# adama-wzr/EffectiveDiffusivityFVM

Hardware: AMD Instinct MI355X
Metric: Mcells*iter/s (Jacobi sweep) at 4096^2 (higher is better)
Workload: dtype f64

## Files before the change

### effectivediffusivityfvm_amd/_capi.py

```python
import ctypes as C
import os

import numpy as np

_PKG = os.path.dirname(os.path.abspath(__file__))
LIB_PATH = os.environ.get("DEFF_AMD_LIB") or os.path.join(_PKG, "libdeff_amd.so")

KERNEL_AUTO, KERNEL_EXPLICIT, KERNEL_SCALAR, KERNEL_MATFREE, KERNEL_MATFREE_TB = range(5)
KERNEL_NAMES = {"auto": 0, "explicit": 1, "scalar": 2, "matfree": 3, "matfree_tb": 4}

SYMBOLS = [
    "deff_version", "deff_last_error", "deff_error_string", "deff_device_count",
    "deff_create", "deff_create_batch", "deff_batch_size", "deff_recommended_batch", "deff_destroy", "deff_mesh", "deff_set_kernel", "deff_get_kernel",
    "deff_set_tuning", "deff_get_plan", "deff_set_image", "deff_synth_image", "deff_get_image",
    "deff_load_jpeg_gray", "deff_free", "deff_assemble_2phase", "deff_assemble_3phase", "deff_flood_fill", "deff_assemble_from_D", "deff_set_system", "deff_get_system",
    "deff_init_linear", "deff_set_field", "deff_get_field", "deff_solve", "deff_solve_batch", "deff_solve_cg", "deff_sweeps",
    "deff_slab_group_create", "deff_slab_group_destroy", "deff_slab_group_layout", "deff_slab_group_set_tuning", "deff_slab_group_get_plan",
    "deff_slab_group_set_image", "deff_slab_group_synth_image", "deff_slab_group_assemble_2phase",
    "deff_slab_group_init_linear", "deff_slab_group_set_field", "deff_slab_group_get_field",
    "deff_slab_group_sweeps", "deff_slab_group_flux", "deff_slab_group_solve",
    "deff_rccl_unique_id", "deff_slab_rank_create", "deff_slab_rank_create_custom", "deff_slab_rank_destroy", "deff_slab_rank_layout",
    "deff_slab_rank_window", "deff_slab_rank_context", "deff_slab_rank_set_tuning", "deff_slab_rank_set_image_window",
    "deff_slab_rank_synth_image", "deff_slab_rank_assemble_3phase", "deff_slab_group_assemble_3phase", "deff_slab_rank_get_field", "deff_slab_rank_sweeps", "deff_slab_rank_solve",
    "deff_solve_stream", "deff_get_slot_field", "deff_debug_tb_stamps", "deff_flux", "deff_residual", "deff_residual_slot", "deff_residual_D", "deff_set_progress", "deff_last_launches", "deff_device_field", "deff_synchronize",
]


class DeffError(RuntimeError):
    def __init__(self, code, msg):
        super().__init__(f"deff_amd error {code}: {msg}")
        self.code = code


class Result(C.Structure):
    _fields_ = [("iters", C.c_int64), ("checks", C.c_int64), ("deff_raw", C.c_double),
                ("conv", C.c_double), ("loop_ms", C.c_double)]


class CGResultC(C.Structure):
    _fields_ = [("iters", C.c_int64), ("rel_residual", C.c_double), ("deff_raw", C.c_double),
                ("loop_ms", C.c_double), ("converged", C.c_int)]


PROGRESS_FN = C.CFUNCTYPE(None, C.c_int64, C.c_double, C.c_double, C.c_void_p)
NEXT_IMAGE_FN = C.CFUNCTYPE(C.c_int, C.c_void_p, C.c_int, C.POINTER(C.c_uint8), C.POINTER(C.c_int64))
IMAGE_DONE_FN = C.CFUNCTYPE(None, C.c_void_p, C.c_int64, C.c_int, C.POINTER(Result))
_cdp = C.POINTER(C.c_double)
# ... 78 lines not shown
    L.deff_slab_group_solve.argtypes = [ctx, C.c_double, C.c_double, C.c_int64, C.c_int64, C.POINTER(Result),
                                        C.c_void_p, C.c_void_p]
    L.deff_rccl_unique_id.argtypes = [C.c_char_p]
    L.deff_slab_rank_create.argtypes = [C.c_int, C.c_int, C.c_int, C.c_int, C.c_int, C.c_char_p, C.POINTER(ctx)]
    L.deff_slab_rank_create_custom.argtypes = [C.c_int, C.c_int, C.c_int, C.c_int, C.c_int, HOST_EXCHANGE_FN,
                                               HOST_ALLGATHER_FN, C.c_void_p, C.POINTER(ctx)]
    L.deff_slab_rank_destroy.argtypes = [ctx]
    L.deff_slab_rank_layout.argtypes = [ctx, ip, ip]
    L.deff_slab_rank_window.argtypes = [ctx, ip, ip]
    L.deff_slab_rank_context.argtypes = [ctx, C.POINTER(ctx)]
    L.deff_slab_rank_set_image_window.argtypes = [ctx, _u8p]
    L.deff_slab_rank_synth_image.argtypes = [ctx, C.c_uint64, C.c_uint64]
    L.deff_slab_rank_assemble_3phase.argtypes = [ctx, C.c_double, C.c_double, C.c_double, C.c_void_p, C.c_double, C.c_double]
    L.deff_slab_group_assemble_3phase.argtypes = [ctx, C.c_double, C.c_double, C.c_double, C.c_void_p, C.c_double, C.c_double]
    L.deff_slab_rank_get_field.argtypes = [ctx, _dp]
    L.deff_slab_rank_sweeps.argtypes = [ctx, C.c_int64, C.c_double, C.POINTER(C.c_float)]
    L.deff_slab_rank_solve.argtypes = [ctx, C.c_double, C.c_double, C.c_int64, C.c_int64, C.POINTER(Result),
                                       C.c_void_p, C.c_void_p]
    L.deff_solve_stream.argtypes = [ctx, C.c_int, C.c_int, C.c_int, C.c_int, C.c_double, C.c_double, C.c_double,
                                    C.c_double, C.c_double, C.c_double, C.c_int64, C.c_int64, NEXT_IMAGE_FN,
                                    IMAGE_DONE_FN, C.c_void_p]
    L.deff_get_slot_field.argtypes = [ctx, C.c_int, _dp]
    L.deff_debug_tb_stamps.argtypes = [ctx, C.c_double, C.c_void_p, C.POINTER(C.c_int)]
    L.deff_device_field.argtypes = [ctx, C.POINTER(C.c_void_p), C.POINTER(C.c_size_t)]
    L.deff_synchronize.argtypes = [ctx]
    _lib = L
    return L


def check(rc):
    if rc != 0:
        raise DeffError(rc, load().deff_last_error().decode("utf-8", "replace"))
```

### effectivediffusivityfvm_amd/csrc/api_core.hip

```cpp
#include "ctx.hpp"
#include <algorithm>
#include "driver/jpeg_gray.hpp"
#include "flood_fill.hpp"


thread_local char g_err[512] = "";

int fail(int code, const char *fmt, ...)
{
    va_list ap;
    va_start(ap, fmt);
    vsnprintf(g_err, sizeof g_err, fmt, ap);
    va_end(ap);
    return code;
}


extern "C" const char *deff_version(void) { return "deff_amd 0.1 (gfx950)"; }
extern "C" const char *deff_last_error(void) { return g_err; }
extern "C" const char *deff_error_string(int code)
{
    switch (code) {
    case DEFF_OK: return "ok";
    case DEFF_EINVAL: return "invalid argument";
// ... 68 lines not shown
        }
    } while (0);
    if (rc != DEFF_OK) return rc;
    resident_chain_ctx_created(device);
    c->chain_counted = true;
    guard.c = nullptr;
    *out = c;
    return DEFF_OK;
}
DEFF_API_CATCH

extern "C" int deff_destroy(deff_ctx *c)
try {
    if (!c) return DEFF_OK;
    (void)hipSetDevice(c->device);
    if (c->stream) (void)hipStreamSynchronize(c->stream);
    void *bufs[] = {c->pix, c->a0, c->c0, c->aW, c->aE, c->aS, c->aN, c->b, c->code, c->lut,
                    c->Dl, c->Dr, c->mf, c->x[0], c->x[1], c->scratch, c->active};
    for (void *p : bufs) if (p) (void)hipFree(p);
    if (c->mf_host) (void)hipHostFree(c->mf_host);
    if (c->q) (void)hipFree(c->q);
    if (c->resid) (void)hipFree(c->resid);
    if (c->tb_dealt) (void)hipFree(c->tb_dealt);
    if (c->res_flags) (void)hipFree(c->res_flags);
    if (c->res_abort) (void)hipFree(c->res_abort);
    if (c->res_backup) (void)hipFree(c->res_backup);
    void *cg_bufs[] = {c->cg_r, c->cg_p[0], c->cg_p[1], c->cg_tab, c->cg_part, c->cg_scal, c->cg_flags};
    for (void *p : cg_bufs) if (p) (void)hipFree(p);
    if (c->cg_ev0) (void)hipEventDestroy(c->cg_ev0);
    if (c->cg_ev1) (void)hipEventDestroy(c->cg_ev1);
    if (c->q_host) (void)hipHostFree(c->q_host);
    if (c->chain_counted) resident_chain_ctx_destroyed(c->device);
    if (c->ev0) (void)hipEventDestroy(c->ev0);
    if (c->ev1) (void)hipEventDestroy(c->ev1);
    if (c->stream) (void)hipStreamDestroy(c->stream);
    delete c;
    return DEFF_OK;
}
DEFF_API_CATCH

extern "C" int deff_mesh(const deff_ctx *c, int *nx, int *ny, double *dx, double *dy)
try {
    if (!c) return fail(DEFF_EINVAL, "ctx is NULL");
    if (nx) *nx = c->nxt;
    if (ny) *ny = c->ny;
    if (dx) *dx = c->dx;
// ... 95 lines not shown
    else if (!strcmp(key, "tb_R")) c->tb_R = value;
    else if (!strcmp(key, "tb_debug_stall")) c->tb_debug_stall = value;
    else if (!strcmp(key, "tb_debug_stall_skip")) c->tb_debug_stall_skip = value;
    else if (!strcmp(key, "res_kt")) c->res_kt = value;
    else if (!strcmp(key, "tb_sym")) c->tb_sym = value;
    else if (!strcmp(key, "tb_launch")) {
        if (value > 1) return fail(DEFF_EINVAL, "tb_launch takes 0 (resident passes where the tiles fit the chip) or 1 (one launch per pass)");
        c->tb_resident = value == 1 ? 0 : 1;
    }
    else if (!strcmp(key, "flux_reduce")) c->flux_reduce = value > 2 ? 0 : value;
    else if (!strcmp(key, "tb_NW")) c->tb_NW = value;
    else if (!strcmp(key, "dict")) c->dict_enabled = value ? 1 : 0;
    else if (!strcmp(key, "tb_xmajor")) c->tb_xmajor = value ? 1 : 0;
    else if (!strcmp(key, "fma")) c->fma = value ? 1 : 0;
    else if (!strcmp(key, "tb_wall_halo")) c->tb_wall_halo = value > 2 ? 2 : value;
    else if (!strcmp(key, "tb_wg")) c->tb_wg = (value + 7) / 8 * 8;
    else if (!strcmp(key, "tb_ranked")) { c->tb_ranked = value ? 1 : 0; c->tb_rank_lost = 0; }
    else if (!strcmp(key, "tb_tall_deal")) c->tb_tall_deal = value ? 1 : 0;
    else if (!strcmp(key, "tb_sym_age")) c->tb_sym_age = value ? 1 : 0;
    else if (!strcmp(key, "tb_sym_shape")) c->tb_sym_shape = value;
    else if (!strcmp(key, "tb_rank_w0")) c->tb_rank_w[0] = value;
    else if (!strcmp(key, "tb_rank_w1")) c->tb_rank_w[1] = value;
    else if (!strcmp(key, "tb_rank_w2")) c->tb_rank_w[2] = value;
    else if (!strcmp(key, "tb_rank_wall")) c->tb_rank_wall = value;
    else return fail(DEFF_EINVAL, "unknown tuning key '%s'", key);
    return DEFF_OK;
}
DEFF_API_CATCH

extern "C" int deff_get_plan(deff_ctx *c, const char *key, int *value)
try {
    if (!c || !key || !value) return fail(DEFF_EINVAL, "NULL argument");
    if (!strcmp(key, "tb_T")) *value = c->plan_T;
    else if (!strcmp(key, "tb_LY")) *value = c->plan_LY;
    else if (!strcmp(key, "tb_strips")) *value = c->plan_ntx;
    else if (!strcmp(key, "tb_chunks_per_image")) *value = c->plan_cpi;
    else if (!strcmp(key, "tb_blocks")) *value = c->plan_blocks;
    else if (!strcmp(key, "tb_impl")) *value = c->plan_impl;
    else if (!strcmp(key, "tb_R")) *value = c->plan_R;
    else if (!strcmp(key, "tb_resident")) *value = c->plan_resident;
    else if (!strcmp(key, "tb_sym")) *value = c->links_sym;
    else if (!strcmp(key, "tb_NW")) *value = c->plan_NW;
    else if (!strcmp(key, "tb_fallbacks")) *value = c->res_fallbacks;
    else if (!strcmp(key, "tb_ranked")) *value = c->plan_ranked;
    else if (!strcmp(key, "tb_aged")) *value = c->plan_aged;
    else if (!strcmp(key, "tb_rank_misses")) *value = c->tb_rank_misses;
    else if (!strcmp(key, "tb_rank_lost")) *value = c->tb_rank_lost;
    else return fail(DEFF_EINVAL, "unknown plan key '%s'", key);
    return DEFF_OK;
}
DEFF_API_CATCH


int image_shape(deff_ctx *c, int W, int H, int ampX, int ampY)
{
    if (W < 1 || H < 1 || ampX < 1 || ampY < 1)
        return fail(DEFF_EINVAL, "image %dx%d / mesh amplification %dx%d invalid", W, H, ampX, ampY);
    if ((long long)W * ampX != c->nxt || (long long)H * ampY != c->ny)
        return fail(DEFF_EINVAL, "image %dx%d x amp %dx%d does not match mesh %dx%d", W, H, ampX, ampY,
                    c->nxt, c->ny);
    if (c->pix && (c->W != W || c->H != H)) { HIP_TRY(hipFree(c->pix)); c->pix = nullptr; }
    TRY(dev_alloc(&c->pix, (size_t)W * H * c->nimg));
    c->W = W; c->H = H; c->ampX = ampX; c->ampY = ampY;
    return DEFF_OK;
}

extern "C" int deff_set_image(deff_ctx *c, const uint8_t *pix, int W, int H, int ampX, int ampY)
try {
    if (!c || !pix) return fail(DEFF_EINVAL, "NULL argument");
    TRY(use_device(c));
// ... 379 lines not shown
```

### effectivediffusivityfvm_amd/csrc/api_solve.hip

```cpp
#include "ctx.hpp"
#include "kernels_dict.hpp"
#include "kernels_sweep.hpp"
#include "kernels_tb.hpp"
#include "kernels_wgtile.hpp"
#include <array>
#include <map>
#include <mutex>



template <class Make> static constexpr auto by_flag(Make make) { return std::array{make(TbTag<false>{}), make(TbTag<true>{})}; }
template <class Make> static constexpr auto by_flags(Make make)
{
    return std::array{make(TbTag<false>{}, TbTag<false>{}), make(TbTag<false>{}, TbTag<true>{}), make(TbTag<true>{}, TbTag<false>{}),
                      make(TbTag<true>{}, TbTag<true>{})};
}
template <class E, size_t... N> static constexpr auto cat(const std::array<E, N> &...parts)
{
    std::array<E, (N + ...)> all{};
    size_t k = 0;
    auto put = [&](const auto &part) { for (const E &e : part) all[k++] = e; };
    (put(parts), ...);
    return all;
}
// ... 494 lines not shown
    if (!found) return DEFF_OK;
    TRY(check_links_symmetric(c));
    if (c->links_sym == 1) *sym = found;
    return DEFF_OK;
}

static int plan_sym(deff_ctx *c, SweepPlan *pl, int T, int own_h, const TileKernel *tile)
{
    pl->impl = 2;
    pl->tile = tile;
    const int lymax = tile->tile_rows() - 2 * T;
    const int cpi = (own_h + lymax - 1) / lymax;
    pl->LY = (own_h + cpi - 1) / cpi;
    pl->tcpi = (own_h + pl->LY - 1) / pl->LY;
    pl->tgy = pl->tcpi * c->nimg;
    const long tiles = (long)pl->ntx * pl->tgy;
    pl->tgx = (int)tiles;
    pl->tblocks = (int)(((tiles + 7) / 8) * 8);
    pl->resident = true;
    TRY(ensure_resident_buffers(c, tiles));
    return DEFF_OK;
}

static int deal_ranked_tiles(deff_ctx *c, SweepPlan *pl, int T, int own_lo, int own_h, int resident, bool *dealt)
{
    *dealt = false;
    int cus = 0;
    HIP_TRY(hipDeviceGetAttribute(&cus, hipDeviceAttributeMultiprocessorCount, c->device));
    const int xcds = 8, per_xcd = cus / xcds, occ = cus > 0 ? resident / cus : 0;
    if (cus % xcds != 0 || occ != 3 || resident != occ * cus) return DEFF_OK;
    const int slots = cus * 4;
    const int ntx = pl->ntx, cap = own_h / (3 * T);
    const int ncol = ntx * c->nimg;
    if (ntx > 0xFFFF || c->nimg > 0x7FFF || ncol > slots) return DEFF_OK;
    const int nq = std::min(slots / ncol, cap);
    if (nq < 1 || c->tb_rank_wall < 1000 || c->tb_rank_w[0] < 1 || c->tb_rank_w[1] < 1 || c->tb_rank_w[2] < 1) return DEFF_OK;
    const std::vector<int> key = {T, own_lo, own_h, ntx, c->nimg, pl->shift, resident, c->tb_rank_w[0], c->tb_rank_w[1], c->tb_rank_w[2], c->tb_rank_wall};
    auto fill_plan = [&]() {
        pl->dealt = c->tb_dealt;
        pl->LY = c->tb_dealt_LY;
        pl->tcpi = 3 * c->tb_dealt_nmax;
        pl->tgy = pl->tcpi * c->nimg;
        pl->tgx = (ntx * pl->tgy + 3) / 4;
        pl->tblocks = resident;
        *dealt = true;
    };
    if (c->tb_dealt && key == c->tb_dealt_key) { fill_plan(); return DEFF_OK; }
    const double v[3] = {(double)c->tb_rank_w[0], (double)c->tb_rank_w[1], (double)c->tb_rank_w[2]};
    const int K = T * (T - 1) + 8;
    std::vector<std::array<double, 3>> speed(ncol, std::array<double, 3>{v[0], v[1], v[2]});
    const bool walls = ntx >= 3;
    if (walls) {
        const int hw = (T + 1) & ~1, wout = TB_COLS - 2 * hw;
        const int last_cols = c->nx - ((ntx - 1) * wout - pl->shift);
        const double extra = c->tb_rank_wall / 1000.0 - 1.0, by_rank[3] = {2.5, 1.5, 1.0};
        const double fill = (double)std::min(last_cols, TB_COLS) / TB_COLS;
        for (int img = 0; img < c->nimg; ++img)
            for (int r = 0; r < 3; ++r) {
                speed[(size_t)img * ntx][r] = v[r] / (1.0 + extra * by_rank[r]);
                speed[(size_t)img * ntx + ntx - 1][r] = v[r] / (1.0 + extra * by_rank[r] * fill);
            }
    }
    struct Strip { int n[3]; int ly[3]; };
    std::vector<Strip> st(ncol);
    for (auto &q : st) q.n[0] = q.n[1] = q.n[2] = nq;
    int spare[3] = {slots - ncol * nq, slots - ncol * nq, slots - ncol * nq};
    auto strip_time = [&](int tx) {
        const Strip &q = st[tx];
        const std::array<double, 3> &u = speed[tx];
        return ((double)T * own_h + (double)K * (q.n[0] + q.n[1] + q.n[2])) / (q.n[0] * u[0] + q.n[1] * u[1] + q.n[2] * u[2]);
    };
    for (int it = 0; it < 3 * slots; ++it) {
        int worst = -1;
        double tw = 0;
        for (int tx = 0; tx < ncol; ++tx) {
            const double t = strip_time(tx);
            if (t > tw) { tw = t; worst = tx; }
        }
        int r = -1;
        for (int k = 0; k < 3; ++k)
            if (spare[k] > 0 && st[worst].n[k] < cap && (r < 0 || spare[k] > spare[r])) r = k;
        if (r < 0) break;
        ++st[worst].n[r];
        --spare[r];
    }
    int nmax = 0;
    for (int tx = 0; tx < ncol; ++tx) {
        Strip &q = st[tx];
        const double t = strip_time(tx);
        int left = own_h;
        for (int r = 2; r >= 1; --r) {
            int ly = (int)((t * speed[tx][r] - K) / T);
            if (ly < T) ly = T;
            q.ly[r] = ly;
            left -= q.n[r] * ly;
        }
        q.ly[0] = (left + q.n[0] - 1) / q.n[0];
        if (q.ly[0] < T) return DEFF_OK;
        nmax = std::max(nmax, std::max(q.n[0], std::max(q.n[1], q.n[2])));
    }
    if ((long)3 * c->nimg * ntx * nmax >= (1L << 30)) return DEFF_OK;
    const size_t entries = (size_t)resident * 4 + 1;
    {
        std::vector<int4> &tab = c->tb_dealt_host;
        tab.assign(entries, make_int4(0, 0, 0, 0));
        auto tile = [&](int r, int col, int q) {
            const Strip &sp = st[col];
            const int img = col / ntx, tx = col % ntx;
            const int own0 = own_lo + img * c->ny;
            const int own_hi = own0 + own_h;
            int ry0 = own0;
            for (int k = 0; k < r; ++k) ry0 += sp.n[k] * sp.ly[k];
            ry0 += q * sp.ly[r];
            int rows_here = std::min(sp.ly[r], own_hi - ry0);
            if (r == 2 && q == sp.n[2] - 1) rows_here = own_hi - ry0;
            return make_int4(tx | (img << 16), ry0, rows_here > 0 ? rows_here : 0, (int)((unsigned)(((r * c->nimg + img) * ntx + tx) * nmax + q) | ((unsigned)r << 30)));
        };
        for (int r = 0; r < 3; ++r) {
            auto slot = [&](int m, int w) { return ((((size_t)(r * per_xcd + m % per_xcd) << 3) | (size_t)(m / per_xcd)) * 4 + w); };
            std::vector<char> used((size_t)cus * 4, 0);
            std::vector<int4> wall_tiles;
            if (walls)
                for (int img = 0; img < c->nimg; ++img)
                    for (int tx : {0, ntx - 1})
                        for (int q = 0; q < st[(size_t)img * ntx + tx].n[r]; ++q) wall_tiles.push_back(tile(r, img * ntx + tx, q));
            const int nw = (int)wall_tiles.size();
            for (int k = 0; k < nw; ++k) {
                int m = (int)(((long)k * cus) / std::max(nw, 1) + (long)r * cus / 3) % cus, w = 0;
                while (used[(size_t)m * 4 + w]) { if (++w == 4) { w = 0; m = (m + 1) % cus; } }
                used[(size_t)m * 4 + w] = 1;
                tab[slot(m, w)] = wall_tiles[k];
            }
            int m = 0, w = 0;
            for (int col = 0; col < ncol; ++col) {
                if (walls && (col % ntx == 0 || col % ntx == ntx - 1)) continue;
                for (int q = 0; q < st[col].n[r]; ++q) {
                    while (m < cus && used[(size_t)m * 4 + w]) { if (++w == 4) { w = 0; ++m; } }
                    if (m >= cus) return fail(DEFF_ESTATE, "dealt tiles: more chunks than waves (rank %d)", r);
                    used[(size_t)m * 4 + w] = 1;
                    tab[slot(m, w)] = tile(r, col, q);
                }
            }
        }
        if (c->tb_dealt_cap < entries) {
            TRY(resident_check(c));
            if (c->tb_dealt) { HIP_TRY(hipStreamSynchronize(c->stream)); HIP_TRY(hipFree(c->tb_dealt)); c->tb_dealt = nullptr; }
            HIP_TRY(hipMalloc((void **)&c->tb_dealt, entries * sizeof(int4)));
            c->tb_dealt_cap = entries;
        }
        HIP_TRY(hipMemcpyAsync(c->tb_dealt, tab.data(), entries * sizeof(int4), hipMemcpyHostToDevice, c->stream));
        HIP_TRY(hipStreamSynchronize(c->stream));
        c->tb_dealt_key = key;
        c->tb_dealt_LY = st[ntx / 2].ly[1];
        c->tb_dealt_nmax = nmax;
        c->tb_dealt_miss_at = (size_t)resident * 4;
        c->tb_dealt_waves = 0;
        c->tb_dealt_looks = 0;
    }
    fill_plan();
    return DEFF_OK;
}

static int plan_streaming(deff_ctx *c, SweepPlan *pl, int T, int own_lo, int own_h)
{
    pl->impl = 1;
    pl->resident = false;
    pl->guard = c->lut_guard;
    int resident = c->tb_wg;
    if (!resident) {
        TRY(resident_blocks(c, STREAMING[tb_index(T)][2 * pl->fma + pl->guard], 256, &resident));
        if (resident < 1) TRY(cu_count(c, &resident));
    }
    pl->dealt = nullptr;
    if (c->tb_ranked && !c->tb_rank_lost && !c->tb_LY && !c->tb_wg && pl->band_h == 0 && !c->slab && T == 8 && !c->masked) {
        bool dealt = false;
        TRY(deal_ranked_tiles(c, pl, T, own_lo, own_h, resident, &dealt));
        if (dealt) return DEFF_OK;
    }
    int LY = c->tb_LY;
    if (!LY) {
        long best_cost = -1;
        const bool top_wall = own_lo == 0;
        for (int k = 1; k <= 8; ++k) {
            const int cpi_max = (int)(((long)k * resident * 4) / ((long)pl->ntx * c->nimg));
            if (cpi_max < 1) continue;
            int ly = (own_h + cpi_max - 1) / cpi_max;
            if (ly < T) ly = T;
            const int cpi = (own_h + ly - 1) / ly;
            const long cost = (long)k * (ly + T + ((cpi > 1 || !top_wall) ? T : 0) + 8);
            if (best_cost < 0 || cost < best_cost) { best_cost = cost; LY = ly; }
        }
        if (!LY) LY = own_h;
    }
    if (LY > own_h) LY = own_h;
    pl->LY = LY;
    pl->tcpi = (own_h + LY - 1) / LY;
    pl->tgy = pl->tcpi * c->nimg;
// ... 155 lines not shown
int enqueue_tb_pass(deff_ctx *c, const SweepPlan &pl)
{
    TRY(launch_tb_pass(c, pl));
    c->cur ^= 1;
    return DEFF_OK;
}

int launch_tb_pass(deff_ctx *c, const SweepPlan &pl)
{
    const double *xin = c->x[c->cur];
    double *xout = c->x[c->cur ^ 1];
    const int flip = c->serpentine ? c->cur : 0;
    const uint8_t *mask = c->masked ? c->active : nullptr;
    const int allb = (c->lut_allb || c->nx != c->nxt) ? 1 : 0;
    if (pl.impl == 2) {
        if (!pl.tile->pass)
            return fail(DEFF_ESTATE, "tiles of %d waves only exist as resident launches (plan again with tb_launch = 1)", pl.tile->NW);
        hipLaunchKernelGGL(pl.tile->pass, dim3(pl.tblocks), dim3(pl.tile->threads()), 0, c->stream, c->lut, c->code, xin, xout, c->nx,
                           c->mesh_ny, c->ny, c->dom_lo, pl.own_lo, pl.own_h, pl.tcpi, pl.LY, mask, pl.ntx, pl.tgy, c->tb_xmajor, allb,
                           c->lut_nrows, pl.shift, pl.omw, c->tb_stamps);
        HIP_TRY(hipPeekAtLastError());
        return DEFF_OK;
    }
    hipLaunchKernelGGL(STREAMING[tb_index(pl.T)][2 * pl.fma + pl.guard], dim3(pl.tblocks), dim3(256), 0, c->stream, c->lut, c->code,
                       xin, xout, c->nx, c->mesh_ny, c->ny, c->dom_lo, pl.own_lo, pl.own_h, pl.tcpi, mask, pl.LY, pl.ntx, pl.tgx, pl.tgy,
                       flip, c->tb_xmajor, allb, c->lut_nrows, pl.shift, pl.omw, c->tb_stamps, pl.dealt);
    HIP_TRY(hipPeekAtLastError());
    if (pl.dealt) c->tb_dealt_waves += (int64_t)pl.tblocks * 4;
    return DEFF_OK;
}

static int launch_resident_passes(deff_ctx *c, const SweepPlan &pl, int64_t *n)
{
    int64_t np = *n / pl.T;
    if (np > 0 && !c->res_pending) {
        TRY(dev_alloc(&c->res_backup, c->n));
        HIP_TRY(hipMemcpyAsync(c->res_backup, c->x[c->cur], sizeof(double) * c->n, hipMemcpyDeviceToDevice, c->stream));
        c->res_backup_cur = c->cur;
        c->res_redo = 0;
        c->res_omega = pl.omega;
    }
    const double pass_s = (double)c->n * pl.T / 0.9e12;
    const int64_t cap = std::max<int64_t>(64, std::min<int64_t>(4096, (int64_t)(25e-3 / pass_s)));
    while (np > 0) {
        const int chunk = (int)(np < cap ? np : cap);
        if (c->res_epoch > (1u << 30)) {
            HIP_TRY(hipMemsetAsync(c->res_flags, 0, sizeof(unsigned) * c->res_flags_n * WGR_FLAG_STRIDE, c->stream));
            c->res_epoch = 0;
        }
        const hipError_t e = launch_resident(c, pl, c->x[c->cur], c->x[c->cur ^ 1], chunk, c->res_epoch);
        if (e != hipSuccess) return fail(DEFF_EHIP, "resident launch failed: %s", hipGetErrorString(e));
// ... 400 lines not shown
```

### effectivediffusivityfvm_amd/csrc/ctx.hpp

```cpp
#pragma once
#include <hip/hip_runtime.h>

#include <algorithm>
#include <cmath>
#include <cstdarg>
#include <cstdio>
#include <cstdlib>
#include <cstring>
#include <new>
#include <string>
#include <vector>

#pragma GCC visibility push(default)
#include "../../include/deff_amd.h"
#pragma GCC visibility pop
#include "fvm_row.hpp"
#include "kernels_setup.hpp"
#include "lut_layout.hpp"

using namespace deff;


extern thread_local char g_err[512];
int fail(int code, const char *fmt, ...) __attribute__((format(printf, 2, 3)));
// ... 95 lines not shown
    int links_sym = 0;
    int tb_sym = 0;
    int tb_debug_stall = 0;
    int tb_debug_stall_skip = 0;
    int plan_resident = 0;
    unsigned *res_flags = nullptr;
    size_t res_flags_n = 0;
    unsigned res_epoch = 0;
    unsigned *res_abort = nullptr;
    bool res_pending = false;
    double *res_backup = nullptr;
    int res_backup_cur = 0;
    int64_t res_redo = 0;
    double res_omega = 0;
    int res_fallbacks = 0;
    bool chain_counted = false;
    int fma = 0;
    int tb_xmajor = 1;
    int tb_tall_deal = 1;
    int plan_aged = 0;
    int tb_sym_age = 1;
    int tb_sym_shape = 0;
    int tb_ranked = 1;
    int tb_rank_w[3] = {460, 325, 215};
    int tb_rank_wall = 1100;
    int4 *tb_dealt = nullptr;
    size_t tb_dealt_cap = 0;
    std::vector<int4> tb_dealt_host;
    std::vector<int> tb_dealt_key;
    size_t tb_dealt_miss_at = 0;
    int64_t tb_dealt_waves = 0;
    int tb_dealt_looks = 0;
    int tb_rank_misses = 0, tb_rank_lost = 0;
    int tb_dealt_LY = 0, tb_dealt_nmax = 0;
    int plan_ranked = 0;
    int64_t last_launches = 0;

    double *cg_r = nullptr, *cg_p[2] = {nullptr, nullptr};
    double *cg_tab = nullptr;
    double *cg_part = nullptr;
    size_t cg_part_cap = 0;
    void *cg_scal = nullptr;
    unsigned *cg_flags = nullptr;
    hipEvent_t cg_ev0 = nullptr, cg_ev1 = nullptr;
};

static inline int use_device(const deff_ctx *c)
{
// ... 160 lines not shown
```

### include/deff_amd.h

```cpp
#ifndef DEFF_AMD_H
#define DEFF_AMD_H

#include <stddef.h>
#include <stdint.h>

#ifdef __cplusplus
extern "C" {
#endif

#define DEFF_OK            0
#define DEFF_EINVAL       -1
#define DEFF_EHIP         -2
#define DEFF_ENOMEM       -3
#define DEFF_ENODEV       -4
#define DEFF_ESTATE       -5
#define DEFF_ECOMM        -6

#define DEFF_KERNEL_AUTO       0
#define DEFF_KERNEL_EXPLICIT   1
#define DEFF_KERNEL_SCALAR     2
#define DEFF_KERNEL_MATFREE    3
#define DEFF_KERNEL_MATFREE_TB 4

typedef struct deff_ctx deff_ctx;
// ... 95 lines not shown
int deff_slab_rank_create(int device, int nx, int NY, int rank, int nranks, const char *id128,
                          deff_slab_rank **out);
typedef int (*deff_host_exchange_fn)(void *user, const double *send_up, double *recv_up, const double *send_down,
                                     double *recv_down, size_t count);
typedef int (*deff_host_allgather_fn)(void *user, const double *mine, double *all, size_t count);
int deff_slab_rank_create_custom(int device, int nx, int NY, int rank, int nranks, deff_host_exchange_fn exchange,
                                 deff_host_allgather_fn allgather, void *user, deff_slab_rank **out);
int deff_slab_rank_destroy(deff_slab_rank *s);
int deff_slab_rank_layout(const deff_slab_rank *s, int *first_row, int *row_count);
int deff_slab_rank_window(const deff_slab_rank *s, int *first_row, int *row_count);
int deff_slab_rank_context(deff_slab_rank *s, deff_ctx **ctx);
int deff_slab_rank_set_tuning(deff_slab_rank *s, const char *key, int value);
int deff_slab_rank_set_image_window(deff_slab_rank *s, const uint8_t *pix_window);
int deff_slab_rank_assemble_3phase(deff_slab_rank *s, double Ds, double Df, double Dg, const unsigned int *Grid_window,
                                   double CL, double CR);
int deff_slab_rank_synth_image(deff_slab_rank *s, uint64_t seed, uint64_t img);
int deff_slab_rank_get_field(deff_slab_rank *s, double *x_own);
int deff_slab_rank_sweeps(deff_slab_rank *s, int64_t n, double omega, float *ms);
int deff_slab_rank_solve(deff_slab_rank *s, double omega, double tol, int64_t max_iter,
                         int64_t check_every, deff_result *out, double *MFL, double *MFR);

int deff_debug_tb_stamps(deff_ctx *ctx, double omega, unsigned long long *out, int *ntiles);

int deff_device_field(deff_ctx *ctx, void **d_x, size_t *row_pitch_bytes);
int deff_synchronize(deff_ctx *ctx);

#ifdef __cplusplus
}
#endif
#endif
```

Measured before the change: 1.264 million.

## Calibrate ranked tile dealing from measured per-XCD wave timings

```diff
diff --git a/effectivediffusivityfvm_amd/_capi.py b/effectivediffusivityfvm_amd/_capi.py
--- a/effectivediffusivityfvm_amd/_capi.py
+++ b/effectivediffusivityfvm_amd/_capi.py
@@ -22,7 +22,7 @@
     "deff_rccl_unique_id", "deff_slab_rank_create", "deff_slab_rank_create_custom", "deff_slab_rank_destroy", "deff_slab_rank_layout",
     "deff_slab_rank_window", "deff_slab_rank_context", "deff_slab_rank_set_tuning", "deff_slab_rank_set_image_window",
     "deff_slab_rank_synth_image", "deff_slab_rank_assemble_3phase", "deff_slab_group_assemble_3phase", "deff_slab_rank_get_field", "deff_slab_rank_sweeps", "deff_slab_rank_solve",
-    "deff_solve_stream", "deff_get_slot_field", "deff_debug_tb_stamps", "deff_flux", "deff_residual", "deff_residual_slot", "deff_residual_D", "deff_set_progress", "deff_last_launches", "deff_device_field", "deff_synchronize",
+    "deff_solve_stream", "deff_get_slot_field", "deff_debug_tb_stamps", "deff_debug_deal", "deff_flux", "deff_residual", "deff_residual_slot", "deff_residual_D", "deff_set_progress", "deff_last_launches", "deff_device_field", "deff_synchronize",
 ]
 
 
@@ -147,6 +147,7 @@
                                     IMAGE_DONE_FN, C.c_void_p]
     L.deff_get_slot_field.argtypes = [ctx, C.c_int, _dp]
     L.deff_debug_tb_stamps.argtypes = [ctx, C.c_double, C.c_void_p, C.POINTER(C.c_int)]
+    L.deff_debug_deal.argtypes = [C.c_void_p, C.c_void_p, C.c_int, C.c_void_p, C.c_int, C.c_void_p, C.c_void_p, C.c_void_p]
     L.deff_device_field.argtypes = [ctx, C.POINTER(C.c_void_p), C.POINTER(C.c_size_t)]
     L.deff_synchronize.argtypes = [ctx]
     _lib = L
diff --git a/effectivediffusivityfvm_amd/csrc/api_core.hip b/effectivediffusivityfvm_amd/csrc/api_core.hip
--- a/effectivediffusivityfvm_amd/csrc/api_core.hip
+++ b/effectivediffusivityfvm_amd/csrc/api_core.hip
@@ -114,6 +114,9 @@
     if (c->q) (void)hipFree(c->q);
     if (c->resid) (void)hipFree(c->resid);
     if (c->tb_dealt) (void)hipFree(c->tb_dealt);
+    if (c->tb_cal_stamps) (void)hipFree(c->tb_cal_stamps);
+    if (c->tb_cal_host) (void)hipHostFree(c->tb_cal_host);
+    if (c->tb_cal_ev) (void)hipEventDestroy(c->tb_cal_ev);
     if (c->res_flags) (void)hipFree(c->res_flags);
     if (c->res_abort) (void)hipFree(c->res_abort);
     if (c->res_backup) (void)hipFree(c->res_backup);
@@ -255,7 +258,10 @@
     else if (!strcmp(key, "tb_rank_w0")) c->tb_rank_w[0] = value;
     else if (!strcmp(key, "tb_rank_w1")) c->tb_rank_w[1] = value;
     else if (!strcmp(key, "tb_rank_w2")) c->tb_rank_w[2] = value;
+    else if (!strcmp(key, "tb_rank_w3")) c->tb_rank_w[3] = value;
     else if (!strcmp(key, "tb_rank_wall")) c->tb_rank_wall = value;
+    else if (!strcmp(key, "tb_rank_cal")) c->tb_rank_cal = value ? 1 : 0;
+    else if (!strcmp(key, "tb_rank_T")) c->tb_rank_T = value ? 1 : 0;
     else return fail(DEFF_EINVAL, "unknown tuning key '%s'", key);
     return DEFF_OK;
 }
@@ -279,6 +285,7 @@
     else if (!strcmp(key, "tb_aged")) *value = c->plan_aged;
     else if (!strcmp(key, "tb_rank_misses")) *value = c->tb_rank_misses;
     else if (!strcmp(key, "tb_rank_lost")) *value = c->tb_rank_lost;
+    else if (!strcmp(key, "tb_rank_cal")) *value = c->tb_cal_state;
     else return fail(DEFF_EINVAL, "unknown plan key '%s'", key);
     return DEFF_OK;
 }
diff --git a/effectivediffusivityfvm_amd/csrc/api_solve.hip b/effectivediffusivityfvm_amd/csrc/api_solve.hip
--- a/effectivediffusivityfvm_amd/csrc/api_solve.hip
+++ b/effectivediffusivityfvm_amd/csrc/api_solve.hip
@@ -540,144 +540,336 @@
     return DEFF_OK;
 }
 
+constexpr int DEAL_XCDS = 8, DEAL_CLASSES = 3;
+constexpr int CAL_SKIP = 1, CAL_LAUNCHES = 3;
+constexpr double CAL_TRUST = 1.5;
+
+struct DealGeom {
+    int cus = 0, occ = 0, T = 0, ntx = 0, nimg = 0, own_lo = 0, own_h = 0, pitch = 0;
+    double last_fill = 1.0;
+    int K() const { return T * (T - 1) + 8; }
+    bool walls() const { return ntx >= 3; }
+    int cls(int tx) const { return !walls() ? 0 : tx == 0 ? 1 : tx == ntx - 1 ? 2 : 0; }
+    size_t nspeed() const { return (size_t)DEAL_XCDS * occ * DEAL_CLASSES; }
+    size_t sidx(int xcd, int r, int k) const { return ((size_t)xcd * occ + r) * DEAL_CLASSES + k; }
+};
+
+static std::vector<double> deal_prior(const DealGeom &g, const int *w, int wall)
+{
+    std::vector<double> v(g.nspeed());
+    const double extra = wall / 1000.0 - 1.0;
+    for (int x = 0; x < DEAL_XCDS; ++x)
+        for (int r = 0; r < g.occ; ++r) {
+            v[g.sidx(x, r, 0)] = w[r];
+            v[g.sidx(x, r, 1)] = w[r] / (1.0 + extra);
+            v[g.sidx(x, r, 2)] = w[r] / (1.0 + extra * g.last_fill);
+        }
+    return v;
+}
+
+static int deal_cut(const DealGeom &g, const std::vector<double> &v, std::vector<int4> &tab, int *nmax_out, int *LY_out)
+{
+    const int T = g.T, K = g.K(), occ = g.occ, cus = g.cus, per_xcd = cus / DEAL_XCDS, ntx = g.ntx;
+    const int slots = cus * 4;
+    const int ncol = ntx * g.nimg;
+    const int cap = g.own_h / (occ * T);
+    if (ncol > slots) return 0;
+    const int nq = std::min(slots / ncol, cap);
+    if (nq < 1) return 0;
+    std::vector<int> n((size_t)ncol * occ);
+    std::vector<double> u((size_t)ncol * occ);
+    for (int col = 0; col < ncol; ++col)
+        for (int r = 0; r < occ; ++r) {
+            double s = 0;
+            for (int x = 0; x < DEAL_XCDS; ++x) s += v[g.sidx(x, r, g.cls(col % ntx))];
+            u[(size_t)col * occ + r] = s / DEAL_XCDS;
+        }
+    auto strip_time = [&](int col) {
+        double nn = 0, sv = 0;
+        for (int r = 0; r < occ; ++r) { nn += n[(size_t)col * occ + r]; sv += n[(size_t)col * occ + r] * u[(size_t)col * occ + r]; }
+        return ((double)T * g.own_h + K * nn) / sv;
+    };
+    int nmax = 0;
+    std::vector<int> where;
+    for (int round = 0; round < 3; ++round) {
+        std::fill(n.begin(), n.end(), nq);
+        std::vector<int> spare(occ, slots - ncol * nq);
+        for (int it = 0; it < occ * slots; ++it) {
+            int worst = -1;
+            double tw = 0;
+            for (int col = 0; col < ncol; ++col) {
+                const double t = strip_time(col);
+                if (t > tw) { tw = t; worst = col; }
+            }
+            int r = -1;
+            for (int k = 0; k < occ; ++k)
+                if (spare[k] > 0 && n[(size_t)worst * occ + k] < cap && (r < 0 || spare[k] > spare[r])) r = k;
+            if (r < 0) break;
+            ++n[(size_t)worst * occ + r];
+            --spare[r];
+        }
+        nmax = *std::max_element(n.begin(), n.end());
+        if ((long)occ * ncol * nmax >= (1L << 30)) return 0;
+        where.assign((size_t)occ * ncol * nmax, -1);
+        for (int r = 0; r < occ; ++r) {
+            auto slot = [&](int m, int w) { return (int)(((((size_t)(r * per_xcd + m % per_xcd) << 3) | (size_t)(m / per_xcd)) * 4 + w)); };
+            std::vector<char> used((size_t)cus * 4, 0);
+            std::vector<int> wall;
+            if (g.walls())
+                for (int img = 0; img < g.nimg; ++img)
+                    for (int tx : {0, ntx - 1})
+                        for (int q = 0; q < n[((size_t)img * ntx + tx) * occ + r]; ++q) wall.push_back((r * ncol + img * ntx + tx) * nmax + q);
+            const int nw = (int)wall.size();
+            for (int k = 0; k < nw; ++k) {
+                int m = (int)(((long)k * cus) / std::max(nw, 1) + (long)r * cus / occ) % cus, w = 0;
+                while (used[(size_t)m * 4 + w]) { if (++w == 4) { w = 0; m = (m + 1) % cus; } }
+                used[(size_t)m * 4 + w] = 1;
+                where[wall[k]] = slot(m, w);
+            }
+            int m = 0, w = 0;
+            for (int col = 0; col < ncol; ++col) {
+                if (g.cls(col % ntx) != 0) continue;
+                for (int q = 0; q < n[(size_t)col * occ + r]; ++q) {
+                    while (m < cus && used[(size_t)m * 4 + w]) { if (++w == 4) { w = 0; ++m; } }
+                    if (m >= cus) return -1;
+                    used[(size_t)m * 4 + w] = 1;
+                    where[((size_t)r * ncol + col) * nmax + q] = slot(m, w);
+                }
+            }
+        }
+        for (int col = 0; col < ncol; ++col)
+            for (int r = 0; r < occ; ++r) {
+                double s = 0;
+                const int nn = n[(size_t)col * occ + r];
+                for (int q = 0; q < nn; ++q) s += v[g.sidx((where[((size_t)r * ncol + col) * nmax + q] >> 2) & 7, r, g.cls(col % ntx))];
+                u[(size_t)col * occ + r] = s / nn;
+            }
+    }
+    tab.assign((size_t)occ * cus * 4 + 1, make_int4(0, 0, 0, 0));
+    int LY = 0;
+    std::vector<int> idx, rows;
+    std::vector<double> vj, h;
+    std::vector<char> fixed;
+    for (int col = 0; col < ncol; ++col) {
+        const int img = col / ntx, tx = col % ntx, k = g.cls(tx);
+        idx.clear();
+        vj.clear();
+        for (int r = 0; r < occ; ++r)
+            for (int q = 0; q < n[(size_t)col * occ + r]; ++q) {
+                const int ci = (r * ncol + col) * nmax + q;
+                if (where[ci] < 0) return -1;
+                idx.push_back(ci);
+                vj.push_back(v[g.sidx((where[ci] >> 2) & 7, r, k)]);
+            }
+        const int nc = (int)idx.size();
+        fixed.assign(nc, 0);
+        h.assign(nc, (double)T);
+        for (bool again = true; again;) {
+            again = false;
+            double rows_free = g.own_h, steps = 0, sv = 0;
+            for (int j = 0; j < nc; ++j) {
+                if (fixed[j]) rows_free -= T;
+                else { steps += K; sv += vj[j]; }
+            }
+            if (sv <= 0) break;
+            const double t = ((double)T * rows_free + steps) / sv;
+            for (int j = 0; j < nc; ++j)
+                if (!fixed[j]) {
+                    h[j] = (t * vj[j] - K) / T;
+                    if (h[j] < T) { fixed[j] = 1; h[j] = T; again = true; }
+                }
+        }
+        rows.assign(nc, 0);
+        int left = g.own_h;
+        for (int j = 0; j < nc; ++j) { rows[j] = std::max(T, (int)std::floor(h[j])); left -= rows[j]; }
+        if (left < 0) return 0;
+        std::vector<int> order(nc);
+        for (int j = 0; j < nc; ++j) order[j] = j;
+        std::stable_sort(order.begin(), order.end(), [&](int a, int b) { return h[a] - std::floor(h[a]) > h[b] - std::floor(h[b]); });
+        for (int j = 0; left > 0; j = (j + 1) % nc, --left) ++rows[order[j]];
+        int y = g.own_lo + img * g.pitch;
+        for (int j = 0; j < nc; ++j) {
+            const int ci = idx[j], r = ci / (ncol * nmax);
+            tab[where[ci]] = make_int4(tx | (img << 16), y, rows[j], (int)((unsigned)ci | ((unsigned)r << 30)));
+            if (col == ntx / 2 && !LY && r == std::min(1, occ - 1)) LY = rows[j];
+            y += rows[j];
+        }
+    }
+    *nmax_out = nmax;
+    *LY_out = LY;
+    return 1;
+}
+
+static int deal_fit(const DealGeom &g, const std::vector<int4> &tab, int nmax, const unsigned long long *st, int nl,
+                    const std::vector<double> &prior, std::vector<double> &v)
+{
+    const size_t per = (size_t)g.occ * g.ntx * g.nimg * nmax, ns = g.nspeed();
+    std::vector<double> work(ns, 0.0), ticks(ns, 0.0);
+    std::vector<char> used(ns, 0);
+    long waves = 0, bad = 0;
+    for (size_t e = 0; e + 1 < tab.size(); ++e) {
+        const int4 d = tab[e];
+        if (d.z <= 0) continue;
+        const int r = (int)((unsigned)d.w >> 30);
+        const size_t si = (size_t)(d.w & 0x3FFFFFFF), k = g.sidx((int)((e >> 2) & 7), r, g.cls(d.x & 0xFFFF));
+        if (si >= per) return 0;
+        used[k] = 1;
+        for (int l = 0; l < nl; ++l) {
+            const unsigned long long s1 = st[2 * (l * per + si) + 1], dur = s1 & 0xFFFFFFFFull;
+            ++waves;
+            if (dur == 0 || (int)((s1 >> 32) & 0xF) != r) { ++bad; continue; }
+            work[k] += (double)g.T * d.z + g.K();
+            ticks[k] += (double)dur;
+        }
+    }
+    if (waves == 0 || bad * 100 > waves) return 0;
+    std::vector<double> fit(ns, 0.0), ratio;
+    for (size_t k = 0; k < ns; ++k) {
+        if (!used[k]) continue;
+        if (ticks[k] <= 0) return 0;
+        fit[k] = work[k] / (ticks[k] / 100.0);
+        ratio.push_back(fit[k] / prior[k]);
+    }
+    std::vector<double> sorted = ratio;
+    std::nth_element(sorted.begin(), sorted.begin() + sorted.size() / 2, sorted.end());
+    const double med = sorted[sorted.size() / 2];
+    for (double q : ratio)
+        if (q >= med * CAL_TRUST || q * CAL_TRUST <= med) return 0;
+    v.assign(ns, 0.0);
+    for (size_t k = 0; k < ns; ++k) v[k] = used[k] ? fit[k] : prior[k] * med;
+    return 1;
+}
+
+static int deal_calibrate(deff_ctx *c, const DealGeom &g)
+{
+    if (c->tb_cal_state != 2) return DEFF_OK;
+    const hipError_t q = hipEventQuery(c->tb_cal_ev);
+    if (q == hipErrorNotReady) return DEFF_OK;
+    HIP_TRY(q);
+    c->tb_cal_state = 4;
+    std::vector<double> v;
+    const std::vector<double> prior = deal_prior(g, c->tb_rank_w, c->tb_rank_wall);
+    if (!deal_fit(g, c->tb_dealt_host, c->tb_dealt_nmax, c->tb_cal_host, CAL_LAUNCHES, prior, v)) return DEFF_OK;
+    std::vector<int4> tab;
+    int nmax = 0, LY = 0;
+    if (deal_cut(g, v, tab, &nmax, &LY) != 1 || tab.size() != c->tb_dealt_host.size()) return DEFF_OK;
+    HIP_TRY(hipMemcpyAsync(c->tb_dealt, tab.data(), (tab.size() - 1) * sizeof(int4), hipMemcpyHostToDevice, c->stream));
+    HIP_TRY(hipStreamSynchronize(c->stream));
+    c->tb_dealt_host.swap(tab);
+    c->tb_dealt_nmax = nmax;
+    c->tb_dealt_LY = LY;
+    c->tb_cal_key = c->tb_dealt_key;
+    c->tb_cal_speed = v;
+    c->tb_cal_state = 3;
+    return DEFF_OK;
+}
+
 static int deal_ranked_tiles(deff_ctx *c, SweepPlan *pl, int T, int own_lo, int own_h, int resident, bool *dealt)
 {
     *dealt = false;
     int cus = 0;
     HIP_TRY(hipDeviceGetAttribute(&cus, hipDeviceAttributeMultiprocessorCount, c->device));
-    const int xcds = 8, per_xcd = cus / xcds, occ = cus > 0 ? resident / cus : 0;
-    if (cus % xcds != 0 || occ != 3 || resident != occ * cus) return DEFF_OK;
-    const int slots = cus * 4;
-    const int ntx = pl->ntx, cap = own_h / (3 * T);
-    const int ncol = ntx * c->nimg;
-    if (ntx > 0xFFFF || c->nimg > 0x7FFF || ncol > slots) return DEFF_OK;
-    const int nq = std::min(slots / ncol, cap);
-    if (nq < 1 || c->tb_rank_wall < 1000 || c->tb_rank_w[0] < 1 || c->tb_rank_w[1] < 1 || c->tb_rank_w[2] < 1) return DEFF_OK;
-    const std::vector<int> key = {T, own_lo, own_h, ntx, c->nimg, pl->shift, resident, c->tb_rank_w[0], c->tb_rank_w[1], c->tb_rank_w[2], c->tb_rank_wall};
+    DealGeom g;
+    g.cus = cus; g.occ = cus > 0 ? resident / cus : 0; g.T = T; g.ntx = pl->ntx; g.nimg = c->nimg;
+    g.own_lo = own_lo; g.own_h = own_h; g.pitch = c->ny;
+    if (cus % DEAL_XCDS != 0 || g.occ < 2 || g.occ > 4 || resident != g.occ * cus) return DEFF_OK;
+    if (g.ntx > 0xFFFF || c->nimg > 0x7FFF || c->tb_rank_wall < 1000) return DEFF_OK;
+    for (int r = 0; r < g.occ; ++r)
+        if (c->tb_rank_w[r] < 1) return DEFF_OK;
+    {
+        const int hw = (T + 1) & ~1, wout = TB_COLS - 2 * hw;
+        const int last_cols = c->nx - ((g.ntx - 1) * wout - pl->shift);
+        g.last_fill = (double)std::min(last_cols, TB_COLS) / TB_COLS;
+    }
+    std::vector<int> key = {T, own_lo, own_h, g.ntx, c->nimg, pl->shift, resident, c->tb_rank_wall, c->tb_rank_cal};
+    for (int r = 0; r < g.occ; ++r) key.push_back(c->tb_rank_w[r]);
     auto fill_plan = [&]() {
         pl->dealt = c->tb_dealt;
         pl->LY = c->tb_dealt_LY;
-        pl->tcpi = 3 * c->tb_dealt_nmax;
+        pl->tcpi = g.occ * c->tb_dealt_nmax;
         pl->tgy = pl->tcpi * c->nimg;
-        pl->tgx = (ntx * pl->tgy + 3) / 4;
+        pl->tgx = (g.ntx * pl->tgy + 3) / 4;
         pl->tblocks = resident;
         *dealt = true;
     };
-    if (c->tb_dealt && key == c->tb_dealt_key) { fill_plan(); return DEFF_OK; }
-    const double v[3] = {(double)c->tb_rank_w[0], (double)c->tb_rank_w[1], (double)c->tb_rank_w[2]};
-    const int K = T * (T - 1) + 8;
-    std::vector<std::array<double, 3>> speed(ncol, std::array<double, 3>{v[0], v[1], v[2]});
-    const bool walls = ntx >= 3;
-    if (walls) {
-        const int hw = (T + 1) & ~1, wout = TB_COLS - 2 * hw;
-        const int last_cols = c->nx - ((ntx - 1) * wout - pl->shift);
-        const double extra = c->tb_rank_wall / 1000.0 - 1.0, by_rank[3] = {2.5, 1.5, 1.0};
-        const double fill = (double)std::min(last_cols, TB_COLS) / TB_COLS;
-        for (int img = 0; img < c->nimg; ++img)
-            for (int r = 0; r < 3; ++r) {
-                speed[(size_t)img * ntx][r] = v[r] / (1.0 + extra * by_rank[r]);
-                speed[(size_t)img * ntx + ntx - 1][r] = v[r] / (1.0 + extra * by_rank[r] * fill);
-            }
-    }
-    struct Strip { int n[3]; int ly[3]; };
-    std::vector<Strip> st(ncol);
-    for (auto &q : st) q.n[0] = q.n[1] = q.n[2] = nq;
-    int spare[3] = {slots - ncol * nq, slots - ncol * nq, slots - ncol * nq};
-    auto strip_time = [&](int tx) {
-        const Strip &q = st[tx];
-        const std::array<double, 3> &u = speed[tx];
-        return ((double)T * own_h + (double)K * (q.n[0] + q.n[1] + q.n[2])) / (q.n[0] * u[0] + q.n[1] * u[1] + q.n[2] * u[2]);
-    };
-    for (int it = 0; it < 3 * slots; ++it) {
-        int worst = -1;
-        double tw = 0;
-        for (int tx = 0; tx < ncol; ++tx) {
-            const double t = strip_time(tx);
-            if (t > tw) { tw = t; worst = tx; }
-        }
-        int r = -1;
-        for (int k = 0; k < 3; ++k)
-            if (spare[k] > 0 && st[worst].n[k] < cap && (r < 0 || spare[k] > spare[r])) r = k;
-        if (r < 0) break;
-        ++st[worst].n[r];
-        --spare[r];
-    }
-    int nmax = 0;
-    for (int tx = 0; tx < ncol; ++tx) {
-        Strip &q = st[tx];
-        const double t = strip_time(tx);
-        int left = own_h;
-        for (int r = 2; r >= 1; --r) {
-            int ly = (int)((t * speed[tx][r] - K) / T);
-            if (ly < T) ly = T;
-            q.ly[r] = ly;
-            left -= q.n[r] * ly;
-        }
-        q.ly[0] = (left + q.n[0] - 1) / q.n[0];
-        if (q.ly[0] < T) return DEFF_OK;
-        nmax = std::max(nmax, std::max(q.n[0], std::max(q.n[1], q.n[2])));
-    }
-    if ((long)3 * c->nimg * ntx * nmax >= (1L << 30)) return DEFF_OK;
-    const size_t entries = (size_t)resident * 4 + 1;
-    {
-        std::vector<int4> &tab = c->tb_dealt_host;
-        tab.assign(entries, make_int4(0, 0, 0, 0));
-        auto tile = [&](int r, int col, int q) {
-            const Strip &sp = st[col];
-            const int img = col / ntx, tx = col % ntx;
-            const int own0 = own_lo + img * c->ny;
-            const int own_hi = own0 + own_h;
-            int ry0 = own0;
-            for (int k = 0; k < r; ++k) ry0 += sp.n[k] * sp.ly[k];
-            ry0 += q * sp.ly[r];
-            int rows_here = std::min(sp.ly[r], own_hi - ry0);
-            if (r == 2 && q == sp.n[2] - 1) rows_here = own_hi - ry0;
-            return make_int4(tx | (img << 16), ry0, rows_here > 0 ? rows_here : 0, (int)((unsigned)(((r * c->nimg + img) * ntx + tx) * nmax + q) | ((unsigned)r << 30)));
-        };
-        for (int r = 0; r < 3; ++r) {
-            auto slot = [&](int m, int w) { return ((((size_t)(r * per_xcd + m % per_xcd) << 3) | (size_t)(m / per_xcd)) * 4 + w); };
-            std::vector<char> used((size_t)cus * 4, 0);
-            std::vector<int4> wall_tiles;
-            if (walls)
-                for (int img = 0; img < c->nimg; ++img)
-                    for (int tx : {0, ntx - 1})
-                        for (int q = 0; q < st[(size_t)img * ntx + tx].n[r]; ++q) wall_tiles.push_back(tile(r, img * ntx + tx, q));
-            const int nw = (int)wall_tiles.size();
-            for (int k = 0; k < nw; ++k) {
-                int m = (int)(((long)k * cus) / std::max(nw, 1) + (long)r * cus / 3) % cus, w = 0;
-                while (used[(size_t)m * 4 + w]) { if (++w == 4) { w = 0; m = (m + 1) % cus; } }
-                used[(size_t)m * 4 + w] = 1;
-                tab[slot(m, w)] = wall_tiles[k];
-            }
-            int m = 0, w = 0;
-            for (int col = 0; col < ncol; ++col) {
-                if (walls && (col % ntx == 0 || col % ntx == ntx - 1)) continue;
-                for (int q = 0; q < st[col].n[r]; ++q) {
-                    while (m < cus && used[(size_t)m * 4 + w]) { if (++w == 4) { w = 0; ++m; } }
-                    if (m >= cus) return fail(DEFF_ESTATE, "dealt tiles: more chunks than waves (rank %d)", r);
-                    used[(size_t)m * 4 + w] = 1;
-                    tab[slot(m, w)] = tile(r, col, q);
-                }
-            }
-        }
-        if (c->tb_dealt_cap < entries) {
-            TRY(resident_check(c));
-            if (c->tb_dealt) { HIP_TRY(hipStreamSynchronize(c->stream)); HIP_TRY(hipFree(c->tb_dealt)); c->tb_dealt = nullptr; }
-            HIP_TRY(hipMalloc((void **)&c->tb_dealt, entries * sizeof(int4)));
-            c->tb_dealt_cap = entries;
-        }
-        HIP_TRY(hipMemcpyAsync(c->tb_dealt, tab.data(), entries * sizeof(int4), hipMemcpyHostToDevice, c->stream));
-        HIP_TRY(hipStreamSynchronize(c->stream));
-        c->tb_dealt_key = key;
-        c->tb_dealt_LY = st[ntx / 2].ly[1];
-        c->tb_dealt_nmax = nmax;
-        c->tb_dealt_miss_at = (size_t)resident * 4;
-        c->tb_dealt_waves = 0;
-        c->tb_dealt_looks = 0;
+    if (c->tb_dealt && key == c->tb_dealt_key) {
+        TRY(deal_calibrate(c, g));
+        fill_plan();
+        return DEFF_OK;
+    }
+    const bool measured = c->tb_rank_cal && key == c->tb_cal_key;
+    std::vector<int4> &tab = c->tb_dealt_host;
+    int nmax = 0, LY = 0;
+    const int rc = deal_cut(g, measured ? c->tb_cal_speed : deal_prior(g, c->tb_rank_w, c->tb_rank_wall), tab, &nmax, &LY);
+    if (rc < 0) return fail(DEFF_ESTATE, "dealt tiles: more chunks than waves");
+    if (rc == 0) return DEFF_OK;
+    const size_t entries = tab.size();
+    if (c->tb_dealt_cap < entries) {
+        TRY(resident_check(c));
+        if (c->tb_dealt) { HIP_TRY(hipStreamSynchronize(c->stream)); HIP_TRY(hipFree(c->tb_dealt)); c->tb_dealt = nullptr; }
+        HIP_TRY(hipMalloc((void **)&c->tb_dealt, entries * sizeof(int4)));
+        c->tb_dealt_cap = entries;
+    }
+    HIP_TRY(hipMemcpyAsync(c->tb_dealt, tab.data(), entries * sizeof(int4), hipMemcpyHostToDevice, c->stream));
+    HIP_TRY(hipStreamSynchronize(c->stream));
+    c->tb_dealt_key = key;
+    c->tb_dealt_LY = LY;
+    c->tb_dealt_nmax = nmax;
+    c->tb_dealt_miss_at = entries - 1;
+    c->tb_dealt_waves = 0;
+    c->tb_dealt_looks = 0;
+    c->tb_cal_state = !c->tb_rank_cal ? 0 : measured ? 3 : 1;
+    c->tb_cal_launch = 0;
+    if (c->tb_cal_state == 1) {
+        c->tb_cal_per = (size_t)g.occ * g.ntx * g.nimg * nmax;
+        const size_t pairs = c->tb_cal_per * CAL_LAUNCHES;
+        if (c->tb_cal_cap < pairs) {
+            if (c->tb_cal_stamps) { HIP_TRY(hipFree(c->tb_cal_stamps)); c->tb_cal_stamps = nullptr; }
+            if (c->tb_cal_host) { HIP_TRY(hipHostFree(c->tb_cal_host)); c->tb_cal_host = nullptr; }
+            c->tb_cal_cap = 0;
+            HIP_TRY(hipMalloc((void **)&c->tb_cal_stamps, pairs * 2 * sizeof(unsigned long long)));
+            HIP_TRY(hipHostMalloc((void **)&c->tb_cal_host, pairs * 2 * sizeof(unsigned long long)));
+            c->tb_cal_cap = pairs;
+        }
+        if (!c->tb_cal_ev) HIP_TRY(hipEventCreateWithFlags(&c->tb_cal_ev, hipEventDisableTiming));
+        HIP_TRY(hipMemsetAsync(c->tb_cal_stamps, 0, pairs * 2 * sizeof(unsigned long long), c->stream));
     }
     fill_plan();
     return DEFF_OK;
 }
+
+extern "C" int deff_debug_deal(const int *geom, const int *w, int wall, const unsigned long long *stamps, int nl, int *tab,
+                               double *speed, int *info)
+try {
+    if (!geom || !w || !tab || !speed || !info || (nl > 0 && !stamps)) return fail(DEFF_EINVAL, "NULL argument");
+    DealGeom g;
+    g.cus = geom[0]; g.occ = geom[1]; g.T = geom[2]; g.ntx = geom[4]; g.nimg = geom[5]; g.own_lo = 0; g.own_h = geom[6]; g.pitch = geom[6];
+    if (g.cus < DEAL_XCDS || g.cus % DEAL_XCDS || g.occ < 2 || g.occ > 4 || g.T < 1 || g.T > 8 || g.ntx < 1 || g.nimg < 1 || g.own_h < 1)
+        return fail(DEFF_EINVAL, "deff_debug_deal: bad geometry");
+    const int hw = (g.T + 1) & ~1, wout = TB_COLS - 2 * hw;
+    g.last_fill = (double)std::min(geom[3] - ((g.ntx - 1) * wout - geom[7]), TB_COLS) / TB_COLS;
+    info[0] = info[1] = info[2] = info[3] = 0;
+    std::vector<double> v = deal_prior(g, w, wall);
+    std::vector<int4> t;
+    int nmax = 0, LY = 0;
+    int rc = deal_cut(g, v, t, &nmax, &LY);
+    if (rc < 0) return fail(DEFF_ESTATE, "dealt tiles: more chunks than waves");
+    if (rc == 1 && nl > 0) {
+        std::vector<double> fit;
+        if (deal_fit(g, t, nmax, stamps, nl, v, fit)) {
+            std::vector<int4> t2;
+            int nmax2 = 0, LY2 = 0;
+            if (deal_cut(g, fit, t2, &nmax2, &LY2) == 1) { t.swap(t2); v = fit; nmax = nmax2; LY = LY2; info[2] = 1; }
+        }
+    }
+    info[0] = rc;
+    info[1] = nmax;
+    info[3] = LY;
+    if (rc == 1) std::memcpy(tab, t.data(), t.size() * sizeof(int4));
+    std::copy(v.begin(), v.end(), speed);
+    return DEFF_OK;
+}
+DEFF_API_CATCH
 
 static int plan_streaming(deff_ctx *c, SweepPlan *pl, int T, int own_lo, int own_h)
 {
@@ -690,7 +882,8 @@
         if (resident < 1) TRY(cu_count(c, &resident));
     }
     pl->dealt = nullptr;
-    if (c->tb_ranked && !c->tb_rank_lost && !c->tb_LY && !c->tb_wg && pl->band_h == 0 && !c->slab && T == 8 && !c->masked) {
+    if (c->tb_ranked && !c->tb_rank_lost && !c->tb_LY && !c->tb_wg && pl->band_h == 0 && !c->slab && (T == 8 || c->tb_rank_T) &&
+        !c->masked) {
         bool dealt = false;
         TRY(deal_ranked_tiles(c, pl, T, own_lo, own_h, resident, &dealt));
         if (dealt) return DEFF_OK;
@@ -892,11 +1085,23 @@
         HIP_TRY(hipPeekAtLastError());
         return DEFF_OK;
     }
+    unsigned long long *stamps = c->tb_stamps;
+    int cal = -1;
+    if (!stamps && pl.dealt && pl.dealt == c->tb_dealt && c->tb_cal_state == 1) {
+        cal = c->tb_cal_launch++ - CAL_SKIP;
+        if (cal >= 0) stamps = c->tb_cal_stamps + (size_t)cal * 2 * c->tb_cal_per;
+    }
     hipLaunchKernelGGL(STREAMING[tb_index(pl.T)][2 * pl.fma + pl.guard], dim3(pl.tblocks), dim3(256), 0, c->stream, c->lut, c->code,
                        xin, xout, c->nx, c->mesh_ny, c->ny, c->dom_lo, pl.own_lo, pl.own_h, pl.tcpi, mask, pl.LY, pl.ntx, pl.tgx, pl.tgy,
-                       flip, c->tb_xmajor, allb, c->lut_nrows, pl.shift, pl.omw, c->tb_stamps, pl.dealt);
+                       flip, c->tb_xmajor, allb, c->lut_nrows, pl.shift, pl.omw, stamps, pl.dealt);
     HIP_TRY(hipPeekAtLastError());
     if (pl.dealt) c->tb_dealt_waves += (int64_t)pl.tblocks * 4;
+    if (cal == CAL_LAUNCHES - 1) {
+        HIP_TRY(hipMemcpyAsync(c->tb_cal_host, c->tb_cal_stamps, sizeof(unsigned long long) * 2 * c->tb_cal_per * CAL_LAUNCHES,
+                               hipMemcpyDeviceToHost, c->stream));
+        HIP_TRY(hipEventRecord(c->tb_cal_ev, c->stream));
+        c->tb_cal_state = 2;
+    }
     return DEFF_OK;
 }
 
diff --git a/effectivediffusivityfvm_amd/csrc/ctx.hpp b/effectivediffusivityfvm_amd/csrc/ctx.hpp
--- a/effectivediffusivityfvm_amd/csrc/ctx.hpp
+++ b/effectivediffusivityfvm_amd/csrc/ctx.hpp
@@ -141,8 +141,16 @@
     int tb_sym_age = 1;
     int tb_sym_shape = 0;
     int tb_ranked = 1;
-    int tb_rank_w[3] = {460, 325, 215};
+    int tb_rank_w[4] = {460, 325, 215, 150};
     int tb_rank_wall = 1100;
+    int tb_rank_cal = 1, tb_rank_T = 0;
+    int tb_cal_state = 0;
+    int tb_cal_launch = 0;
+    size_t tb_cal_per = 0, tb_cal_cap = 0;
+    unsigned long long *tb_cal_stamps = nullptr, *tb_cal_host = nullptr;
+    hipEvent_t tb_cal_ev = nullptr;
+    std::vector<int> tb_cal_key;
+    std::vector<double> tb_cal_speed;
     int4 *tb_dealt = nullptr;
     size_t tb_dealt_cap = 0;
     std::vector<int4> tb_dealt_host;
diff --git a/include/deff_amd.h b/include/deff_amd.h
--- a/include/deff_amd.h
+++ b/include/deff_amd.h
@@ -141,6 +141,9 @@
 
 int deff_debug_tb_stamps(deff_ctx *ctx, double omega, unsigned long long *out, int *ntiles);
 
+int deff_debug_deal(const int *geom, const int *w, int wall, const unsigned long long *stamps, int nl, int *tab,
+                    double *speed, int *info);
+
 int deff_device_field(deff_ctx *ctx, void **d_x, size_t *row_pitch_bytes);
 int deff_synchronize(deff_ctx *ctx);
 
```

Result: faster. 1.281 million (median of 6 runs) (+1.3%).
